# ziniuwan/maed

Measured on AMD Instinct MI355X. Metric: video-clips/sec (BxT frames) train step, higher is better.
Workload: dtype bf16

## Files before the change

include/maed_hip.h:

```cpp
#ifndef MAED_HIP_H
#define MAED_HIP_H

#include <stddef.h>
#include <stdint.h>

#ifdef __cplusplus
extern "C" {
#endif

typedef enum { MAED_F32 = 0, MAED_BF16 = 1,
               MAED_F32X3 = 2, MAED_F32X6 = 3,
               MAED_F32X1 = 4 } maed_dtype;

typedef enum {
    MAED_OK = 0,
    MAED_ERR_ARG = -1,
    MAED_ERR_SHAPE = -2,
    MAED_ERR_ALIGN = -3,
    MAED_ERR_LAUNCH = -4,
    MAED_ERR_UNSUPPORTED = -5
} maed_status;

typedef enum {
    MAED_EPI_STORE = 0,
    MAED_EPI_GELU = 1,
    MAED_EPI_RESID_F32 = 2,
    MAED_EPI_MUL_DGELU = 3,
    MAED_EPI_ATOMIC_F32 = 4,
    MAED_EPI_STORE_F32 = 5,
    MAED_EPI_TANH = 6,
    MAED_EPI_ADD = 7
} maed_epilogue;

typedef enum { MAED_IMPL_AUTO = 0, MAED_IMPL_VALU = 1, MAED_IMPL_MFMA = 2,
               MAED_IMPL_MFMA_GLDS1 = 3, MAED_IMPL_MFMA_GLDS2 = 4,
               MAED_IMPL_MFMA_LONG = 5,
               MAED_IMPL_MFMA_256 = 6,
               MAED_IMPL_X1 = 9,
               MAED_IMPL_MFMA_SK = 10,
               MAED_IMPL_X3 = 7, MAED_IMPL_X6 = 8
} maed_impl;

const char* maed_last_error(void);
int maed_version(void);

typedef enum {
    MAED_OPT_F32_MATMUL = 0,
    MAED_OPT_SIDE_STREAM = 1,
    MAED_OPT_TN_TARGET_WGS = 2,
    MAED_OPT_ABLATE = 3,
    MAED_OPT_GN_BWD_ONEPASS = 4,
    MAED_OPT_F32_BWD_X1 = 5,
    MAED_OPT_ST_FUSED = 6,
    MAED_OPT_CONV3X3_ROWS_WGS = 7,
    MAED_OPT_STEM_WGRAD_WGS = 8,
    MAED_OPT_LBS_FRAMES = 9,
    MAED_OPT_TN_DMA = 10,
    MAED_OPT_X3_PLANES = 11,
    MAED_OPT_X3_PLANES_LN = 12,
    MAED_OPT_SK = 13,
    MAED_OPT_SK_GRID = 14,
    MAED_OPT_TN_SK = 15,
    MAED_OPT_CONV3X3_NARROW_WGS = 16,
    MAED_OPT_CONV3X3_FRAME = 17,
    MAED_OPT_COUNT
} maed_option;
int maed_init(int device);
int maed_device_faults(void);
int maed_device_faults_clear(void);
int maed_set_option(int key, int value);
int maed_get_option(int key);

int maed_layernorm_fwd(const float* x, int64_t x_row_stride, const float* gamma, const float* beta,
                       void* y, int dtype, float* mean, float* rstd,
                       int64_t rows, int C, float eps, void* stream);
int maed_layernorm_bwd(const void* dy, int dtype, const float* x, int64_t x_row_stride,
                       const float* gamma, const float* mean, const float* rstd,
                       const float* dres_in, float* dx_out, void* dx_twin, float* dgamma, float* dbeta,
                       int64_t rows, int C, void* stream);

int maed_gemm_nt(const void* A, int64_t lda, const void* B, int64_t ldb,
                 int64_t M, int64_t N, int64_t K, int dtype, int epilogue,
                 const float* bias, void* out, int64_t ldo, void* out2,
                 const void* aux, int64_t ldaux, int splitk, int impl, void* stream);

int maed_gemm_nt_planes(const void* a_hi, const void* a_lo, int64_t lda, const void* b_hi, const void* b_lo, int64_t ldb, int64_t M, int64_t N, int64_t K,
                        int epilogue, const float* bias, void* out, int64_t ldo, void* out2_bf16, const void* aux, int64_t ldaux, void* out_hi, void* out_lo,
                        int variant, void* stream);
int maed_split_planes(const float* x, void* hi, void* lo, int64_t n, void* stream);

int maed_gemm_tn_wgrad(const void* Y, int64_t ldy, const void* X, int64_t ldx, int64_t M, int N, int K,
                       float* dW, int64_t ldw, float* dbias, int dtype, void* stream);

int maed_transpose_cast(const void* in, int in_dtype, int64_t ldi, int64_t M, int64_t N,
                        void* out_t, int64_t ldt, void* out_c, int64_t ldc, float* colsum,
                        int dtype, void* stream);

int maed_attn_spatial_fwd(const void* qkv, void* o, float* lse, int F, int P, int H, float scale,
                          int dtype, int impl, void* stream);
int maed_attn_spatial_bwd(const void* qkv, const void* o, const void* d_o, const float* lse,
                          void* dqkv, int accumulate, int F, int P, int H, float scale,
                          int dtype, int impl, void* stream);

int maed_attn_temporal_fwd(const void* qkv, void* o, float* lse, int F, int P, int H, int T,
                           float scale, int dtype, void* stream);
int maed_attn_temporal_bwd(const void* qkv, const void* o, const void* d_o, const float* lse,
                           void* dqkv, int accumulate, int F, int P, int H, int T, float scale,
                           int dtype, void* stream);

int maed_st_colmean(const void* x_s, const void* x_t, void* means, float* ws, int F, int P, int C, int dtype, void* stream);
int maed_st_mix_fwd(const void* x_s, const void* x_t, const float* logits, void* mix,
                    int F, int P, int C, int dtype, void* stream);
int maed_st_mix_bwd_reduce(const void* dmix, const void* x_s, const void* x_t, const float* logits,
                           void* dlogits, float* ws, int F, int P, int C, int dtype, void* stream);
int maed_st_mix_bwd_apply(const void* dmix, const float* logits, const void* dmeans, void* dx_s, void* dx_t,
                          int F, int P, int C, int dtype, void* stream);
int maed_st_fused_supported(int P, int C, int dtype);
int maed_st_fused_fwd(const void* x_s, const void* x_t, const void* w_ts, const float* b_ts, void* means, float* logits, void* mix,
                      uint32_t* sync, float* ex, int F, int P, int C, int dtype, void* stream);
int maed_st_fused_bwd(const void* dmix, const void* x_s, const void* x_t, const float* logits, const void* wt_ts, void* dlogits, void* dx_s,
                      void* dx_t, uint32_t* sync, float* ex, int F, int P, int C, int dtype, void* stream);


int maed_embed_add_fwd(const void* patch, int dtype, const float* cls, const float* pos, const float* temp,
                       float* tokens, int F, int P, int C, int T, void* stream);
int maed_embed_add_bwd(const float* dtokens, void* dpatch, int dtype, float* dpos, float* dtemp, int F, int P, int C, int T, void* stream);

int maed_dropout(const float* x, float* y, int64_t n, float p, uint64_t seed, void* stream);
typedef struct { float lr, bias_corr1, bias_corr2, reserved0; uint64_t seed; uint64_t reserved1; } maed_train_state;
int maed_dropout_dev(const float* x, float* y, int64_t n, float p, const maed_train_state* state, uint64_t call_id, void* stream);
int maed_tanh_bwd(const float* dy, const void* y, void* dx, int64_t n, int dtype, void* stream);

typedef struct {
    int F, P, C, H, T, hidden;
    int dtype;
    int impl;
    float eps;
} maed_block_dims;

typedef struct {
    const float *ln1_g, *ln1_b, *ln2_g, *ln2_b;
    const void *w_qkv, *w_ts, *w_proj, *w_fc1, *w_fc2;
    const float *b_qkv, *b_ts, *b_proj, *b_fc1, *b_fc2;
    const void *wt_qkv, *wt_ts, *wt_proj, *wt_fc1, *wt_fc2;
} maed_block_params;

typedef struct {
// ... 163 lines not shown
```

maed_amd/_lib.py:

```python
import ctypes as C
import os

HERE = os.path.dirname(os.path.abspath(__file__))
LIB_PATH = os.environ.get("MAED_HIP_LIB") or os.path.join(HERE, "libmaed_hip.so")

F32, BF16 = 0, 1
F32X3, F32X6, F32X1 = 2, 3, 4
EPI_STORE, EPI_GELU, EPI_RESID_F32, EPI_MUL_DGELU, EPI_ATOMIC_F32, EPI_STORE_F32, EPI_TANH, EPI_ADD = range(8)
IMPL_AUTO, IMPL_VALU, IMPL_MFMA = 0, 1, 2
IMPL_MFMA_256 = 6
IMPL_MFMA_LONG = 5
IMPL_MFMA_SK = 10
IMPL_X3, IMPL_X6, IMPL_X1 = 7, 8, 9
(OPT_F32_MATMUL, OPT_SIDE_STREAM, OPT_TN_TARGET_WGS, OPT_ABLATE, OPT_GN_BWD_ONEPASS, OPT_F32_BWD_X1, OPT_ST_FUSED, OPT_CONV3X3_ROWS_WGS, OPT_STEM_WGRAD_WGS,
 OPT_LBS_FRAMES, OPT_TN_DMA, OPT_X3_PLANES, OPT_X3_PLANES_LN, OPT_SK, OPT_SK_GRID, OPT_TN_SK, OPT_CONV3X3_NARROW_WGS, OPT_CONV3X3_FRAME) = range(18)

vp, i64, i32, f32 = C.c_void_p, C.c_int64, C.c_int, C.c_float


class GnAffineItem(C.Structure):
    _fields_ = [("ab", C.c_void_p), ("dgamma", C.c_void_p), ("dbeta", C.c_void_p), ("N", C.c_int), ("C", C.c_int)]


class BlockDims(C.Structure):
    _fields_ = [("F", i32), ("P", i32), ("C", i32), ("H", i32), ("T", i32), ("hidden", i32),
                ("dtype", i32), ("impl", i32), ("eps", f32)]


_PARAM_FIELDS = ["ln1_g", "ln1_b", "ln2_g", "ln2_b", "w_qkv", "w_ts", "w_proj", "w_fc1", "w_fc2",
                 "b_qkv", "b_ts", "b_proj", "b_fc1", "b_fc2", "wt_qkv", "wt_ts", "wt_proj", "wt_fc1", "wt_fc2"]
_GRAD_FIELDS = _PARAM_FIELDS[:14]


class BlockParams(C.Structure):
    _fields_ = [(n, vp) for n in _PARAM_FIELDS]


class BlockGrads(C.Structure):
    _fields_ = [(n, vp) for n in _GRAD_FIELDS]


class SmplParams(C.Structure):
    _fields_ = [(n, vp) for n in ["v_template", "shapedirs", "posedirs", "J_template", "J_shapedirs", "lbs_weights", "parents"]]


class KtdPtrs(C.Structure):
    _fields_ = [("w", vp * 26), ("b", vp * 26), ("gw", vp * 26), ("gb", vp * 26)]


class LossWeights(C.Structure):
    _fields_ = [(n, f32) for n in ["w_kp2d", "w_kp3d", "w_pose", "w_shape", "w_norm"]]


KTD_W_ANC = 3420

SIGNATURES = {
    "maed_last_error": (C.c_char_p, []),
    "maed_version": (i32, []),
    "maed_init": (i32, [i32]),
    "maed_device_faults": (i32, []),
    "maed_device_faults_clear": (i32, []),
    "maed_set_option": (i32, [i32, i32]),
    "maed_get_option": (i32, [i32]),
    "maed_layernorm_fwd": (i32, [vp, i64, vp, vp, vp, i32, vp, vp, i64, i32, f32, vp]),
    "maed_layernorm_bwd": (i32, [vp, i32, vp, i64, vp, vp, vp, vp, vp, vp, vp, vp, i64, i32, vp]),
    "maed_gemm_tn_wgrad": (i32, [vp, i64, vp, i64, i64, i32, i32, vp, i64, vp, i32, vp]),
    "maed_gemm_nt": (i32, [vp, i64, vp, i64, i64, i64, i64, i32, i32, vp, vp, i64, vp, vp, i64, i32, i32, vp]),
    "maed_transpose_cast": (i32, [vp, i32, i64, i64, i64, vp, i64, vp, i64, vp, i32, vp]),
    "maed_attn_spatial_fwd": (i32, [vp, vp, vp, i32, i32, i32, f32, i32, i32, vp]),
    "maed_attn_spatial_bwd": (i32, [vp, vp, vp, vp, vp, i32, i32, i32, i32, f32, i32, i32, vp]),
    "maed_attn_temporal_fwd": (i32, [vp, vp, vp, i32, i32, i32, i32, f32, i32, vp]),
    "maed_attn_temporal_bwd": (i32, [vp, vp, vp, vp, vp, i32, i32, i32, i32, i32, f32, i32, vp]),
    "maed_st_colmean": (i32, [vp, vp, vp, vp, i32, i32, i32, i32, vp]),
    "maed_st_mix_fwd": (i32, [vp, vp, vp, vp, i32, i32, i32, i32, vp]),
    "maed_st_mix_bwd_reduce": (i32, [vp, vp, vp, vp, vp, vp, i32, i32, i32, i32, vp]),
    "maed_st_mix_bwd_apply": (i32, [vp, vp, vp, vp, vp, i32, i32, i32, i32, vp]),
    "maed_st_fused_supported": (i32, [i32, i32, i32]),
    "maed_st_fused_fwd": (i32, [vp, vp, vp, vp, vp, vp, vp, vp, vp, i32, i32, i32, i32, vp]),
    "maed_st_fused_bwd": (i32, [vp, vp, vp, vp, vp, vp, vp, vp, vp, vp, i32, i32, i32, i32, vp]),
    "maed_embed_add_fwd": (i32, [vp, i32, vp, vp, vp, vp, i32, i32, i32, i32, vp]),
    "maed_embed_add_bwd": (i32, [vp, vp, i32, vp, vp, i32, i32, i32, i32, vp]),
    "maed_ste_block_saved_bytes": (C.c_size_t, [C.POINTER(BlockDims)]),
    "maed_ste_block_scratch_bytes": (C.c_size_t, [C.POINTER(BlockDims)]),
    "maed_gemm_nt_planes": (i32, [vp, vp, i64, vp, vp, i64, i64, i64, i64, i32, vp, vp, i64, vp, vp, i64, vp, vp, i32, vp]),
    "maed_split_planes": (i32, [vp, vp, vp, i64, vp]),
    "maed_ste_block_twin_work_bytes": (C.c_size_t, [C.POINTER(BlockDims)]),
    "maed_ste_block_fwd_twin": (i32, [C.POINTER(BlockDims), C.POINTER(BlockParams), vp, vp, vp, vp, i32, vp]),
    "maed_ste_block_twin_join": (i32, [vp]),
    "maed_ste_block_fwd": (i32, [C.POINTER(BlockDims), C.POINTER(BlockParams), vp, vp, vp, vp]),
    "maed_ste_block_infer": (i32, [C.POINTER(BlockDims), C.POINTER(BlockParams), vp, vp, vp, vp]),
    "maed_ste_block_bwd": (i32, [C.POINTER(BlockDims), C.POINTER(BlockParams), C.POINTER(BlockGrads), vp, vp, vp, vp, vp, vp, vp, vp]),
    "maed_loss_accl_fwd_bwd": (i32, [vp, vp, i32, i32, f32, vp, vp, vp]),
    "maed_dropout": (i32, [vp, vp, i64, f32, C.c_uint64, vp]),
    "maed_dropout_dev": (i32, [vp, vp, i64, f32, vp, C.c_uint64, vp]),
    "maed_tanh_bwd": (i32, [vp, vp, vp, i64, i32, vp]),
    "maed_stream_fence": (i32, [vp, vp]),
    "maed_prof_enable": (i32, [i32]),
    "maed_prof_ntags": (i32, []),
# ... 23 lines not shown
    "maed_gn_affine_grad_batch": (i32, [vp, i32, vp]),
    "maed_comm_load": (i32, [C.c_char_p]),
    "maed_comm_unique_id": (i32, [vp]),
    "maed_comm_init": (i32, [i32, i32, vp]),
    "maed_comm_allreduce_async": (i32, [vp, C.c_size_t, i32, vp]),
    "maed_comm_wait": (i32, [vp]),
    "maed_comm_world": (i32, []),
    "maed_comm_destroy": (i32, []),
    "maed_conv3x3_fwd": (i32, [vp, vp, vp, vp, i32, i32, i32, i32, i32, i32, i32, i32, i32, i32, vp, i32, i32, vp, vp]),
    "maed_conv1x1_fwd": (i32, [vp, i64, vp, i64, i64, i32, i32, vp, i64, i32, vp, i32, vp]),
    "maed_conv3x3_tapmask": (i32, [vp, i32, i32, i32, vp]),
    "maed_conv3x3_s2_dgrad": (i32, [vp, vp, vp, vp, i32, i32, i32, i32, i32, i32, i32, i32, i32, i32, vp]),
    "maed_conv3x3_s2_tables": (i32, [vp, vp, i32, i32, i32, i32, i32, i32, i32, vp]),
    "maed_conv3x3_s2_wgrad": (i32, [vp, vp, vp, vp, vp, vp, i32, i32, i32, i32, i32, i32, i32, i32, vp]),
    "maed_conv3x3_wgrad": (i32, [vp, vp, vp, vp, vp, i32, i32, i32, i32, i32, i32, vp]),
    "maed_eval_pose_errors": (i32, [vp, vp, i32, i32, vp, vp, vp, vp, vp]),
    "maed_similarity_transform": (i32, [vp, vp, i32, i32, vp, vp]),
    "maed_eval_accel": (i32, [vp, vp, i32, i32, vp, vp]),
    "maed_eval_vertex_error": (i32, [vp, vp, i32, i32, vp, vp]),
    "maed_maxpool3s2_same_fwd": (i32, [vp, vp, vp, i32, i32, i32, i32, i32, vp]),
    "maed_maxpool3s2_same_bwd": (i32, [vp, vp, vp, i32, i32, i32, i32, i32, vp]),
    "maed_stem_input": (i32, [vp, vp, i32, i32, i32, i32, i32, i32, i32, i32, i32, i32, vp]),
    "maed_conv3x3_wgrad_rows64_scratch_floats": (i32, [i32, i32, i32, i32, i32]),
    "maed_conv3x3_wgrad_rows64": (i32, [vp, vp, vp, vp, i32, i32, i32, i32, vp]),
    "maed_stem7x7s2_supported": (i32, [i32, i32]),
    "maed_stem7x7s2_fwd": (i32, [vp, vp, vp, vp, vp, i32, i32, i32, i32, vp]),
    "maed_stem7x7s2_wgrad_scratch_floats": (i32, [i32, i32, i32]),
    "maed_stem7x7s2_wgrad": (i32, [vp, vp, vp, vp, i32, i32, i32, i32, vp]),
    "maed_subsample2_fwd": (i32, [vp, vp, i32, i32, i32, i32, i32, vp]),
    "maed_subsample2_bwd": (i32, [vp, vp, i32, i32, i32, i32, i32, vp]),
    "maed_weight_refresh": (i32, [vp, i32, i32, i32, vp]),
    "maed_adam_step": (i32, [vp, vp, vp, vp, vp, i64, f32, f32, f32, f32, f32, f32, f32, f32, vp]),
    "maed_adam_step_dev": (i32, [vp, vp, vp, vp, vp, i64, vp, f32, f32, f32, f32, f32, vp]),
}

_lib = None
_init_pending = False


class MaedHipError(RuntimeError):
    pass


def lib():
    global _lib, _init_pending
    if _lib is None:
        if not os.path.exists(LIB_PATH):
            raise MaedHipError(f"{LIB_PATH} is missing: build it with `python -m maed_amd.build` "
                               "(hipcc --offload-arch=gfx950).  maed_amd has no non-HIP fallback.")
        handle = C.CDLL(LIB_PATH)
        for name, (res, args) in SIGNATURES.items():
            fn = getattr(handle, name)
            fn.restype, fn.argtypes = res, args
        _lib = handle
        apply_options(handle)
        _init_pending = True
    if _init_pending:
        import torch
        if torch.cuda.is_available() and torch.cuda.is_initialized():
            _init_pending = False
            check(_lib.maed_init(torch.cuda.current_device()), "maed_init")
    return _lib


_OPTIONS = {
    OPT_F32_MATMUL: {"exact": 0, "0": 0, "bf16x3": 1, "1": 1, "bf16x6": 2, "2": 2}[os.environ.get("MAED_F32_MATMUL", "exact")],
    OPT_SIDE_STREAM: int(os.environ.get("MAED_WGRAD_SIDE_STREAM", "1") == "1"),
    OPT_TN_TARGET_WGS: int(os.environ.get("MAED_TN_TARGET_WGS", "0")),
    OPT_ABLATE: int(os.environ.get("MAED_GEMM_ABLATE", "0")),
    OPT_F32_BWD_X1: int(os.environ.get("MAED_F32_BWD", "") == "bf16x1"),
    OPT_ST_FUSED: int(os.environ.get("MAED_ST_FUSED", "1")),
    OPT_GN_BWD_ONEPASS: int(os.environ.get("MAED_GN_BWD_ONEPASS", "1")),
    OPT_CONV3X3_ROWS_WGS: 0 if os.environ.get("MAED_CONV3X3_WGRAD_ROWS", "1") == "0" else int(os.environ.get("MAED_CONV3X3_ROWS_WGS", "256")),
    OPT_STEM_WGRAD_WGS: int(os.environ.get("MAED_STEM_WGS", "512")),
    OPT_LBS_FRAMES: int(os.environ.get("MAED_LBS_FB", "0")),
    OPT_TN_DMA: int(os.environ.get("MAED_TN_DMA", "1")),
    OPT_X3_PLANES: int(os.environ.get("MAED_X3_PLANES", "6")),
    OPT_SK: int(os.environ.get("MAED_SK", "1")),
    OPT_SK_GRID: int(os.environ.get("MAED_SK_GRID", "0")),
    OPT_CONV3X3_FRAME: int(os.environ.get("MAED_CONV3X3_FRAME", "1")),
    OPT_CONV3X3_NARROW_WGS: int(os.environ.get("MAED_CONV3X3_NARROW_WGS", "0")),
    OPT_TN_SK: int(os.environ.get("MAED_TN_SK", "1")),
    OPT_X3_PLANES_LN: int(os.environ.get("MAED_X3_PLANES_LN", "0")),
}


def apply_options(handle):
    for k, v in _OPTIONS.items():
        if handle.maed_set_option(k, v) != 0:
            raise MaedHipError(f"maed_set_option({k}, {v}) failed")


def set_option(key, value):
    _OPTIONS[key] = int(value)
    if _lib is not None:
        check(_lib.maed_set_option(key, int(value)), "set_option")


def get_option(key):
    return _OPTIONS[key]


def check(rc, what=""):
    if rc != 0:
        msg = lib().maed_last_error().decode("utf-8", "replace")
        raise MaedHipError(f"{what or 'libmaed_hip'} failed with status {rc}: {msg}")


def device_faults():
    return 0 if _lib is None else int(_lib.maed_device_faults())


def loaded_path():
    return LIB_PATH if _lib is not None else None
```

maed_amd/csrc/gemm.hip:

```cpp
#include "common.cuh"
#include "gemm_epilogue.cuh"
#include "gemm_x3.h"

template <int EPI, typename T>
__global__ __launch_bounds__(256) void gemm_nt_valu_kernel(const T* __restrict__ A, int64_t lda, const T* __restrict__ B,
                                                           int64_t ldb, int64_t M, int64_t N, int64_t K, int64_t k_per_split,
                                                           EpiArgs e) {
    __shared__ float As[16][64 + 1];
    __shared__ float Bs[16][64 + 1];
    const int tid = threadIdx.x;
    const int64_t m0 = (int64_t)blockIdx.y * 64, n0 = (int64_t)blockIdx.x * 64;
    const int64_t kbeg = (int64_t)blockIdx.z * k_per_split;
    const int64_t kend = (kbeg + k_per_split < K) ? kbeg + k_per_split : K;
    const int ty = tid >> 4, tx = tid & 15;
    const int lr = tid >> 2, lk = (tid & 3) * 4;
    float acc[4][4];
#pragma unroll
    for (int i = 0; i < 4; ++i)
#pragma unroll
        for (int j = 0; j < 4; ++j) acc[i][j] = 0.f;
    const int64_t ar = (m0 + lr < M) ? m0 + lr : M - 1;
    const int64_t br = (n0 + lr < N) ? n0 + lr : N - 1;
    const bool vec = sizeof(T) == 4 && (lda % 4 == 0) && (ldb % 4 == 0) && (((uintptr_t)A | (uintptr_t)B) & 15) == 0 && (kbeg % 4 == 0);
    float va[4], vb[4];
// ... 595 lines not shown
    MAED_CHECK_ARG(is_aligned(dy, 16) && is_aligned(wt_image, 16) && is_aligned(zero_page, 16) && is_aligned(dx, 16), MAED_ERR_ALIGN, "conv3x3_s2_dgrad: 16-B alignment");
    MAED_CHECK_ARG((uint64_t)F * H * W * Cin * 2 < (1ull << 32) && (uint64_t)F * Ho * Wo * Cout * 2 < (1ull << 32), MAED_ERR_SHAPE, "conv3x3_s2_dgrad: tensor larger than 4 GB");
    if (F == 0) return MAED_OK;
    const int64_t N = Cin;
    const bool narrow = N <= 64;
    const int tn = narrow ? 1 : (int)((N + GM_BN - 1) / GM_BN);
    EpiArgs e{nullptr, dx, (int64_t)Cin, nullptr, nullptr, (int64_t)Cin};
    for (int py = 0; py < 2; ++py)
        for (int px = 0; px < 2; ++px) {
            const int Ha = (H - py + 1) / 2, Wb = (W - px + 1) / 2;
            if (Ha <= 0 || Wb <= 0) continue;
            const int ey = (py + pad_top) & 1, ex = (px + pad_left) & 1;
            const int nty = ey ? 1 : 2, ntx = ex ? 1 : 2;
            const int base_y = (py + pad_top - ey) / 2 - (nty - 1), base_x = (px + pad_left - ex) / 2 - (ntx - 1);
            Conv3x3Dims d{F, Ho, Wo, Cout, Ha, Wb, 1, -base_y, -base_x, (int64_t)Cout, (int64_t)Cin * Cout, 0};
            d.nty = nty; d.ntx = ntx; d.ky0 = ey + 2 * (nty - 1); d.kx0 = ex + 2 * (ntx - 1); d.o_h = H; d.o_w = W; d.o_py = py; d.o_px = px;
            const int64_t M = (int64_t)F * Ha * Wb;
            const dim3 grid((unsigned)(((M + GM_BM - 1) / GM_BM) * tn));
            if (narrow) hipLaunchKernelGGL((conv3x3_glds_bf16_kernel<MAED_EPI_STORE, true, false, true>), grid, dim3(256), 0, (hipStream_t)stream, (const bf16*)dy,
                                           (const bf16*)wt_image, (const bf16*)zero_page, d, M, N, tn, e);
            else hipLaunchKernelGGL((conv3x3_glds_bf16_kernel<MAED_EPI_STORE, false, false, true>), grid, dim3(256), 0, (hipStream_t)stream, (const bf16*)dy,
                                    (const bf16*)wt_image, (const bf16*)zero_page, d, M, N, tn, e);
        }
    MAED_CHECK_LAUNCH("conv3x3_s2_dgrad");
    return MAED_OK;
}

__global__ __launch_bounds__(256) void bias_fill_kernel(float* __restrict__ out, int64_t ldo, const float* __restrict__ bias, int64_t M, int64_t N) {
    const int64_t i = (int64_t)blockIdx.x * 256 + threadIdx.x;
    if (i < M * N) { const int64_t r = i / N, c = i % N; out[r * ldo + c] = bias ? bias[c] : 0.f; }
}

template <int EPI, typename T>
static int launch_valu(const void* A, int64_t lda, const void* B, int64_t ldb, int64_t M, int64_t N, int64_t K,
                       const EpiArgs& e, int splitk, hipStream_t s) {
    int64_t kps = (K + splitk - 1) / splitk;
    kps = (kps + 15) / 16 * 16;
    const int z = (int)((K + kps - 1) / kps);
    dim3 grid((unsigned)((N + 63) / 64), (unsigned)((M + 63) / 64), (unsigned)z);
    hipLaunchKernelGGL((gemm_nt_valu_kernel<EPI, T>), grid, dim3(256), 0, s, (const T*)A, lda, (const T*)B, ldb, M, N, K, kps, e);
    return MAED_OK;
}

template <int EPI>
static int launch_mfma(const void* A, int64_t lda, const void* B, int64_t ldb, int64_t M, int64_t N, int64_t K,
                       const EpiArgs& e, int splitk, hipStream_t s) {
    const int tm = (int)((M + GM_BM - 1) / GM_BM), tn = (int)((N + GM_BN - 1) / GM_BN);
    const int nkt = (int)(K / GM_BK);
    int kps = (nkt + splitk - 1) / splitk;
    if (kps < 1) kps = 1;
    const int z = (nkt + kps - 1) / kps;
    dim3 grid((unsigned)(tm * tn), 1, (unsigned)z);
    hipLaunchKernelGGL((gemm_nt_mfma_bf16_kernel<EPI>), grid, dim3(256), 0, s, (const bf16*)A, lda, (const bf16*)B, ldb,
                       M, N, K, tn, kps, e);
    return MAED_OK;
}

template <int EPI, int NBUF, bool GN = false>
static int launch_glds(const void* A, int64_t lda, const void* B, int64_t ldb, int64_t M, int64_t N, int64_t K,
                       const EpiArgs& e, int splitk, hipStream_t s) {
    const int tm = (int)((M + GM_BM - 1) / GM_BM), tn = (int)((N + GM_BN - 1) / GM_BN);
    const int nkt = (int)(K / GM_BK);
    int kps = (nkt + splitk - 1) / splitk;
    if (kps < 1) kps = 1;
    const int z = (nkt + kps - 1) / kps;
#ifdef MAED_GEMM_ABLATE
    hipLaunchKernelGGL((gemm_nt_glds_bf16_kernel<EPI, NBUF, GN>), dim3((unsigned)(tm * tn), 1, (unsigned)z), dim3(256), 0, s, (const bf16*)A, lda,
                       (const bf16*)B, ldb, M, N, K, tn, kps, e, maed_opt(MAED_OPT_ABLATE));
#else
    hipLaunchKernelGGL((gemm_nt_glds_bf16_kernel<EPI, NBUF, GN>), dim3((unsigned)(tm * tn), 1, (unsigned)z), dim3(256), 0, s, (const bf16*)A, lda,
                       (const bf16*)B, ldb, M, N, K, tn, kps, e);
#endif
    return MAED_OK;
}

bool maed_gemm_nt_256_launch(int epilogue, const void* A, int64_t lda, const void* B, int64_t ldb, int64_t M, int64_t N, int64_t K, const EpiArgs& e,
                             hipStream_t s);

bool maed_gemm_nt_sk_shape_ok(int64_t M, int64_t N, int64_t K);
bool maed_gemm_nt_sk_launch(int epilogue, const void* A, int64_t lda, const void* B, int64_t ldb, int64_t M, int64_t N, int64_t K, const EpiArgs& e,
                            int mode, int grid_opt, hipStream_t s);
int maed_sk_cus(void);

template <int EPI>
static int dispatch(const void* A, int64_t lda, const void* B, int64_t ldb, int64_t M, int64_t N, int64_t K, int dtype,
                    const EpiArgs& e, int splitk, int impl, hipStream_t s) {
    if (dtype == MAED_F32) {
        MAED_CHECK_ARG(impl == MAED_IMPL_AUTO || impl == MAED_IMPL_VALU || impl == MAED_IMPL_X3 || impl == MAED_IMPL_X6 || impl == MAED_IMPL_X1, MAED_ERR_UNSUPPORTED,
                       "gemm_nt: f32 runs on the exact-f32 VALU kernel (MAED_IMPL_VALU) or the split-bf16 MFMA kernel (MAED_IMPL_X3 / _X6); impl=%d", impl);
        const int np = impl == MAED_IMPL_X3 ? 2 : impl == MAED_IMPL_X6 ? 3 : impl == MAED_IMPL_X1 ? 1 : impl == MAED_IMPL_AUTO ? maed_x3_planes() : 0;
        if (np) {
            const bool ok = maed_x3_nt_shape_ok(A, lda, B, ldb, K);
            const int64_t tiles128 = ((M + 127) / 128) * ((N + 127) / 128);
            if constexpr (EPI == MAED_EPI_STORE || EPI == MAED_EPI_STORE_F32) {
                if (ok && impl != MAED_IMPL_AUTO && splitk == 1 && tiles128 < 48 && K >= 256 && e.ldo >= N && !e.twin && !e.lo && !e.out2_bf16) {
                    int sk = (int)(256 / tiles128);
                    if (sk > K / 32) sk = (int)(K / 32);
                    if (sk > 1) {
                        hipLaunchKernelGGL(bias_fill_kernel, dim3((unsigned)((M * N + 255) / 256)), dim3(256), 0, s, (float*)e.out, e.ldo, e.bias, M, N);
                        EpiArgs ea = e;
                        ea.bias = nullptr;
                        return maed_gemm_nt_x3_launch(MAED_EPI_ATOMIC_F32, np, A, lda, B, ldb, M, N, K, ea, sk, s);
                    }
                }
            }
            if (ok && (impl != MAED_IMPL_AUTO || tiles128 >= 48 || EPI == MAED_EPI_ATOMIC_F32))
                return maed_gemm_nt_x3_launch(EPI, np, A, lda, B, ldb, M, N, K, e, splitk, s);
        }
        if constexpr (EPI == MAED_EPI_STORE || EPI == MAED_EPI_STORE_F32) {
            const int64_t tiles = ((M + 63) / 64) * ((N + 63) / 64);
            if (splitk == 1 && tiles < 96 && K >= 256 && !e.twin && !e.lo && !e.out2_bf16) {
                constexpr int target = 256;
                int sk = (int)(target / tiles);
                if (sk > K / 64) sk = (int)(K / 64);
                if (sk > 1) {
                    hipLaunchKernelGGL(bias_fill_kernel, dim3((unsigned)((M * N + 255) / 256)), dim3(256), 0, s, (float*)e.out, e.ldo, e.bias, M, N);
                    EpiArgs ea{nullptr, e.out, e.ldo, nullptr, nullptr, 0};
                    if (np && maed_x3_nt_shape_ok(A, lda, B, ldb, K)) {
                        const int64_t t128 = ((M + 127) / 128) * ((N + 127) / 128);
                        int sk3 = (int)(256 / t128);
                        if (sk3 > K / 64) sk3 = (int)(K / 64);
                        if (sk3 >= 1) return maed_gemm_nt_x3_launch(MAED_EPI_ATOMIC_F32, np, A, lda, B, ldb, M, N, K, ea, sk3, s);
                    }
                    return launch_valu<MAED_EPI_ATOMIC_F32, float>(A, lda, B, ldb, M, N, K, ea, sk, s);
                }
            }
        }
        return launch_valu<EPI, float>(A, lda, B, ldb, M, N, K, e, splitk, s);
    }
    const bool fits32 = (uint64_t)M * (uint64_t)lda * 2 < (1ull << 32) && (uint64_t)N * (uint64_t)ldb * 2 < (1ull << 32);
    const bool mfma_ok = (K % GM_BK == 0) && (lda % 8 == 0) && (ldb % 8 == 0) && is_aligned(A, 16) && is_aligned(B, 16);
    if (impl == MAED_IMPL_VALU) return launch_valu<EPI, bf16>(A, lda, B, ldb, M, N, K, e, splitk, s);
    if (impl == MAED_IMPL_MFMA_GLDS1 || impl == MAED_IMPL_MFMA_GLDS2) {
        MAED_CHECK_ARG(mfma_ok && fits32, MAED_ERR_ALIGN, "gemm_nt(glds): need K%%64==0 (K=%lld), lda/ldb%%8==0, 16-B aligned A/B", (long long)K);
        return impl == MAED_IMPL_MFMA_GLDS1 ? launch_glds<EPI, 1>(A, lda, B, ldb, M, N, K, e, splitk, s)
                                            : launch_glds<EPI, 2>(A, lda, B, ldb, M, N, K, e, splitk, s);
    }
    const bool ok256 = mfma_ok && fits32 && K >= 128 && splitk == 1 && EPI != MAED_EPI_ATOMIC_F32;
    if (impl == MAED_IMPL_MFMA_256) {
        MAED_CHECK_ARG(ok256, MAED_ERR_ALIGN, "gemm_nt(256): need K%%64==0, K>=128 (K=%lld), lda/ldb%%8==0, 16-B aligned A/B, no split-K", (long long)K);
        maed_gemm_nt_256_launch(EPI, A, lda, B, ldb, M, N, K, e, s);
        return MAED_OK;
    }
    const bool oksk = ok256 && maed_gemm_nt_sk_shape_ok(M, N, K) && !e.gn_sums;
    if (impl == MAED_IMPL_MFMA_SK) {
        const int mode = maed_opt(MAED_OPT_SK);
        MAED_CHECK_ARG(oksk && maed_gemm_nt_sk_launch(EPI, A, lda, B, ldb, M, N, K, e, mode == 0 ? 1 : mode, maed_opt(MAED_OPT_SK_GRID), s), MAED_ERR_ALIGN,
                       "gemm_nt(sk): need K%%128==0 (K=%lld), M, N >= 256, lda/ldb%%8==0, 16-B aligned A/B, no split-K, the library's slab allocation", (long long)K);
        return MAED_OK;
    }
    if (impl == MAED_IMPL_MFMA) {
        MAED_CHECK_ARG(mfma_ok, MAED_ERR_ALIGN, "gemm_nt(mfma): need K%%64==0 (K=%lld), lda/ldb%%8==0, 16-B aligned A/B", (long long)K);
        return launch_mfma<EPI>(A, lda, B, ldb, M, N, K, e, splitk, s);
    }
    if (!mfma_ok) return launch_valu<EPI, bf16>(A, lda, B, ldb, M, N, K, e, splitk, s);
    if constexpr (EPI != MAED_EPI_ATOMIC_F32) {
        const int64_t tiles256 = ((M + 255) / 256) * ((N + 255) / 256);
        const int skmode = maed_opt(MAED_OPT_SK);
        if (oksk && skmode != 0 && tiles256 * 10 >= (int64_t)maed_sk_cus() * 7 &&
            maed_gemm_nt_sk_launch(EPI, A, lda, B, ldb, M, N, K, e, skmode, maed_opt(MAED_OPT_SK_GRID), s))
            return MAED_OK;
        if (ok256 && N >= 256 && tiles256 >= 180 && (K >= 1024 || tiles256 <= 256)) {
            maed_gemm_nt_256_launch(EPI, A, lda, B, ldb, M, N, K, e, s);
            return MAED_OK;
        }
    }
    if constexpr (EPI == MAED_EPI_ATOMIC_F32) return launch_mfma<EPI>(A, lda, B, ldb, M, N, K, e, splitk, s);
    else return fits32 ? launch_glds<EPI, 1>(A, lda, B, ldb, M, N, K, e, splitk, s) : launch_mfma<EPI>(A, lda, B, ldb, M, N, K, e, splitk, s);
}

extern "C" int maed_conv1x1_fwd(const void* x, int64_t ldx, const void* w, int64_t ldw, int64_t M, int Cout, int Cin, void* y, int64_t ldy, int hw,
                                double* gn_sums, int dtype, void* stream) {
    MAED_CHECK_ARG(x && w && y, MAED_ERR_ARG, "conv1x1_fwd: null pointer");
    const int np_call = maed_x3_take_dtype(dtype);
    MAED_CHECK_ARG(dtype == MAED_BF16 || dtype == MAED_F32, MAED_ERR_ARG, "conv1x1_fwd: bad dtype %d", dtype);
    MAED_CHECK_ARG(is_aligned(x, 16) && is_aligned(w, 16) && is_aligned(y, 16), MAED_ERR_ALIGN, "conv1x1_fwd: 16-B alignment");
    MAED_CHECK_ARG(!gn_sums || gn_stats_shape_ok(Cout, hw), MAED_ERR_SHAPE, "conv1x1_fwd: GroupNorm statistics need Cout = 32 * 2^k >= 64 and hw >= 128 (Cout=%d hw=%d)", Cout, hw);
    EpiArgs e{nullptr, y, ldy, nullptr, nullptr, 0, gn_sums, hw};
    if (dtype == MAED_F32) {
        const int x3np = np_call ? np_call : maed_x3_planes();
        MAED_CHECK_ARG(x3np, MAED_ERR_UNSUPPORTED, "conv1x1_fwd: f32 needs the split-bf16 matmul mode (maed_set_option(MAED_OPT_F32_MATMUL, 1 or 2))");
        MAED_CHECK_ARG(M >= 0 && Cout > 0 && Cin > 0 && ldx >= Cin && ldw >= Cin && ldy >= Cout && ldy % 4 == 0 && maed_x3_nt_shape_ok(x, ldx, w, ldw, Cin), MAED_ERR_SHAPE,
                       "conv1x1_fwd(f32): need Cin %% 32 == 0 and 4-element aligned strides (Cin=%d Cout=%d)", Cin, Cout);
        if (M == 0) return MAED_OK;
        MAED_PROPAGATE(maed_conv1x1_x3_launch(x3np, x, ldx, w, ldw, M, Cout, Cin, e, gn_sums != nullptr, (hipStream_t)stream));
        MAED_CHECK_LAUNCH("conv1x1_fwd(x3)");
        return MAED_OK;
    }
    MAED_CHECK_ARG(M >= 0 && Cout > 0 && Cin > 0 && Cin % GM_BK == 0 && ldx >= Cin && ldw >= Cin && ldy >= Cout && ldx % 8 == 0 && ldw % 8 == 0, MAED_ERR_SHAPE,
                   "conv1x1_fwd: need Cin %% 64 == 0 and 8-element aligned strides (Cin=%d Cout=%d)", Cin, Cout);
    MAED_CHECK_ARG((uint64_t)M * (uint64_t)ldx * 2 < (1ull << 32), MAED_ERR_SHAPE, "conv1x1_fwd: activation larger than 4 GB");
    if (M == 0) return MAED_OK;
    if (gn_sums) launch_glds<MAED_EPI_STORE, 1, true>(x, ldx, w, ldw, M, Cout, Cin, e, 1, (hipStream_t)stream);
    else launch_glds<MAED_EPI_STORE, 1>(x, ldx, w, ldw, M, Cout, Cin, e, 1, (hipStream_t)stream);
    MAED_CHECK_LAUNCH("conv1x1_fwd");
    return MAED_OK;
}

int maed_gemm_nt_twin(const void* A, int64_t lda, const void* B, int64_t ldb, int64_t M, int64_t N, int64_t K,
                      int dtype, int epilogue, const float* bias, void* out, int64_t ldo, void* out2,
                      const void* aux, int64_t ldaux, int splitk, int impl, void* stream, void* twin, bool out2_bf16, void* lo);
extern "C" int maed_gemm_nt(const void* A, int64_t lda, const void* B, int64_t ldb, int64_t M, int64_t N, int64_t K,
                            int dtype, int epilogue, const float* bias, void* out, int64_t ldo, void* out2,
                            const void* aux, int64_t ldaux, int splitk, int impl, void* stream) {
    return maed_gemm_nt_twin(A, lda, B, ldb, M, N, K, dtype, epilogue, bias, out, ldo, out2, aux, ldaux, splitk, impl, stream, nullptr, false, nullptr);
}
int maed_gemm_nt_twin(const void* A, int64_t lda, const void* B, int64_t ldb, int64_t M, int64_t N, int64_t K,
                      int dtype, int epilogue, const float* bias, void* out, int64_t ldo, void* out2,
                      const void* aux, int64_t ldaux, int splitk, int impl, void* stream, void* twin, bool out2_bf16, void* lo) {
    MAED_CHECK_ARG(A && B && (out || (twin && lo)), MAED_ERR_ARG, "gemm_nt: null pointer");
    MAED_CHECK_ARG(!lo || (twin && is_aligned(lo, 16)), MAED_ERR_ARG, "gemm_nt: a lo plane goes with the twin (hi) plane, 16-byte aligned");
    {
        const int np_call = maed_x3_take_dtype(dtype);
        if (np_call && impl == MAED_IMPL_AUTO) impl = np_call == 2 ? MAED_IMPL_X3 : np_call == 1 ? MAED_IMPL_X1 : MAED_IMPL_X6;
    }
    MAED_CHECK_ARG(dtype == MAED_F32 || dtype == MAED_BF16, MAED_ERR_ARG, "gemm_nt: bad dtype %d", dtype);
    MAED_CHECK_ARG(M >= 0 && N > 0 && K > 0 && lda >= K && ldb >= K && ldo >= N, MAED_ERR_SHAPE, "gemm_nt: bad extents M=%lld N=%lld K=%lld", (long long)M, (long long)N, (long long)K);
    if (splitk < 1) splitk = 1;
    MAED_CHECK_ARG(splitk == 1 || epilogue == MAED_EPI_ATOMIC_F32, MAED_ERR_ARG, "gemm_nt: split-K needs the atomic epilogue");
    if (M == 0) return MAED_OK;
    MAED_CHECK_ARG(!(twin || out2_bf16) || (dtype == MAED_F32 && (epilogue == MAED_EPI_STORE || epilogue == MAED_EPI_GELU) && N % 8 == 0 && ldo % 8 == 0
                                           && is_aligned(twin, 16) && (!out2_bf16 || is_aligned(out2, 16))),
                   MAED_ERR_ARG, "gemm_nt: twin outputs go with fp32 operands, the STORE / GELU epilogues, N and ldo multiples of 8 and 16-byte aligned buffers");
    EpiArgs e{bias, out, ldo, out2, aux, ldaux};
    e.twin = twin; e.out2_bf16 = out2_bf16; e.lo = lo;
    hipStream_t s = (hipStream_t)stream;
    int rc;
    switch (epilogue) {
        case MAED_EPI_STORE: rc = dispatch<MAED_EPI_STORE>(A, lda, B, ldb, M, N, K, dtype, e, splitk, impl, s); break;
        case MAED_EPI_GELU:
            rc = dispatch<MAED_EPI_GELU>(A, lda, B, ldb, M, N, K, dtype, e, splitk, impl, s); break;
        case MAED_EPI_RESID_F32:
            MAED_CHECK_ARG(aux, MAED_ERR_ARG, "gemm_nt: RESID epilogue needs aux");
            rc = dispatch<MAED_EPI_RESID_F32>(A, lda, B, ldb, M, N, K, dtype, e, splitk, impl, s); break;
        case MAED_EPI_MUL_DGELU:
            MAED_CHECK_ARG(aux, MAED_ERR_ARG, "gemm_nt: MUL_DGELU epilogue needs aux");
            rc = dispatch<MAED_EPI_MUL_DGELU>(A, lda, B, ldb, M, N, K, dtype, e, splitk, impl, s); break;
        case MAED_EPI_ATOMIC_F32: rc = dispatch<MAED_EPI_ATOMIC_F32>(A, lda, B, ldb, M, N, K, dtype, e, splitk, impl, s); break;
// ... 12 lines not shown
```

maed_amd/csrc/options.hip:

```cpp
#include "common.cuh"
#include "gemm_x3.h"
#include <atomic>
#include <string.h>

static std::atomic<int> g_opt[MAED_OPT_COUNT] = {
    {0},
    {1},
    {0},
    {0},
    {1},
    {0},
    {1},
    {256},
    {512},
    {0},
    {1},
    {6},
    {0},
    {1},
    {0},
    {1},
    {0},
    {1},
};

extern "C" int maed_init(int device) {
#ifndef MAED_HOSTSIM
    hipDeviceProp_t prop;
    if (hipGetDeviceProperties(&prop, device) != hipSuccess) { (void)hipGetLastError(); maed_set_error("init: no HIP device %d", device); return MAED_ERR_ARG; }
    if (!strstr(prop.gcnArchName, "gfx950")) {
        maed_set_error("init: device %d is %s; libmaed_hip is built for gfx950 (MI355X) only", device, prop.gcnArchName);
        return MAED_ERR_UNSUPPORTED;
    }
#else
    (void)device;
#endif
    (void)maed_fault_word();
#ifndef MAED_HOSTSIM
    if (maed_init_runtime() != MAED_OK) { maed_set_error("init: could not create the library's side streams / event rings"); return MAED_ERR_LAUNCH; }
#endif
    return MAED_OK;
}

static std::atomic<uint32_t*> g_fault{nullptr};
static std::atomic<int> g_fault_told{0};
uint32_t* maed_fault_word(void) {
    uint32_t* w = g_fault.load(std::memory_order_acquire);
    if (w) return w;
#ifdef MAED_HOSTSIM
    uint32_t* n = (uint32_t*)calloc(16, sizeof(uint32_t));
#else
    uint32_t* n = nullptr;
    if (hipHostMalloc((void**)&n, 64, hipHostMallocMapped | hipHostMallocCoherent) != hipSuccess || !n) { (void)hipGetLastError(); return nullptr; }
    memset(n, 0, 64);
#endif
    uint32_t* expected = nullptr;
    if (!g_fault.compare_exchange_strong(expected, n, std::memory_order_acq_rel)) {
#ifdef MAED_HOSTSIM
        free(n);
#else
        (void)hipHostFree(n);
#endif
        return expected;
    }
    return n;
}
bool maed_fault_seen(const char* who) {
    uint32_t* w = g_fault.load(std::memory_order_acquire);
    if (!w || *(volatile uint32_t*)w == 0) return false;
    if (!g_fault_told.exchange(1))
        maed_set_error("%s: %u frame-barrier timeout(s) on this device (workgroups of a frame were not co-resident: shared GPU / preemption); the affected results were "
                       "NaN-poisoned, the one-pass GroupNorm backward and the fused attentive addition now run as their multi-launch forms", who, *(volatile uint32_t*)w);
    return true;
}
extern "C" int maed_device_faults(void) {
    uint32_t* w = g_fault.load(std::memory_order_acquire);
    const int n = w ? (int)*(volatile uint32_t*)w : 0;
    if (n > 0)
        maed_set_error("%d frame-barrier timeout(s) on this device (workgroups of a frame were not co-resident: shared GPU / preemption); the affected results were "
                       "NaN-poisoned, the one-pass GroupNorm backward and the fused attentive addition run as their multi-launch forms from the next call on", n);
    return n;
}
extern "C" int maed_device_faults_clear(void) { uint32_t* w = g_fault.load(std::memory_order_acquire); if (w) *(volatile uint32_t*)w = 0; g_fault_told.store(0); return MAED_OK; }

extern "C" int maed_set_option(int key, int value) {
    MAED_CHECK_ARG(key >= 0 && key < MAED_OPT_COUNT, MAED_ERR_ARG, "set_option: unknown option %d", key);
    if (key == MAED_OPT_F32_MATMUL) MAED_CHECK_ARG(value >= 0 && value <= 2, MAED_ERR_ARG, "set_option: MAED_OPT_F32_MATMUL takes 0 (exact), 1 (bf16x3) or 2 (bf16x6)");
    if (key == MAED_OPT_TN_TARGET_WGS) MAED_CHECK_ARG(value == 0 || value >= 64, MAED_ERR_ARG, "set_option: MAED_OPT_TN_TARGET_WGS must be 0 (heuristic) or >= 64");
    if (key == MAED_OPT_CONV3X3_ROWS_WGS || key == MAED_OPT_STEM_WGRAD_WGS) MAED_CHECK_ARG(value >= 0 && value <= 65535, MAED_ERR_ARG, "set_option: workgroup count out of range");
    if (key == MAED_OPT_LBS_FRAMES) MAED_CHECK_ARG(value == 0 || value == 4 || value == 8 || value == 16, MAED_ERR_ARG, "set_option: MAED_OPT_LBS_FRAMES takes 0 (auto), 4, 8 or 16");
    if (key == MAED_OPT_X3_PLANES) MAED_CHECK_ARG(value == 0 || (value >= 2 && value <= 7 && value != 3), MAED_ERR_ARG, "set_option: MAED_OPT_X3_PLANES takes 0 (fp32 operands) or a kernel variant 2, 4, 5, 6, 7");
    if (key == MAED_OPT_SK) MAED_CHECK_ARG(value >= 0 && value <= 3, MAED_ERR_ARG, "set_option: MAED_OPT_SK takes 0 (off), 1 (heuristic), 2 (no K cuts) or 3 (always)");
    if (key == MAED_OPT_TN_SK) MAED_CHECK_ARG(value == 0 || value == 1, MAED_ERR_ARG, "set_option: MAED_OPT_TN_SK takes 0 or 1");
    if (key == MAED_OPT_SK_GRID) MAED_CHECK_ARG(value >= 0 && value <= 512, MAED_ERR_ARG, "set_option: MAED_OPT_SK_GRID takes 0 (one workgroup per CU) or a workgroup count <= 512");
    g_opt[key].store(value, std::memory_order_relaxed);
    return MAED_OK;
}

extern "C" int maed_get_option(int key) {
    if (key < 0 || key >= MAED_OPT_COUNT) { maed_set_error("get_option: unknown option %d", key); return MAED_ERR_ARG; }
    return g_opt[key].load(std::memory_order_relaxed);
}

int maed_opt(int key) { return g_opt[key].load(std::memory_order_relaxed); }

int maed_x3_planes(void) {
    const int v = maed_opt(MAED_OPT_F32_MATMUL);
    return v == 1 ? 2 : v == 2 ? 3 : 0;
}
```

Measured before the change: 409.7.

## Add persistent panel GEMM kernel keeping A K-panel resident in LDS

Adds a persistent MFMA bf16 NT GEMM. Each workgroup owns a contiguous run of 128x128 output tiles and keeps the full A row-panel (K up to 512) in LDS, so A is loaded once per tile row while B slices stream through a 4-deep DMA ring. It is selected automatically for short-K GEMMs with simple epilogues when there are at least as many tiles as CUs. The aim is to cut redundant A global loads and launch/tail overhead for the transformer's small-K matmuls, at the cost of large LDS use (one workgroup per CU) and possible load imbalance.

```diff
diff --git a/include/maed_hip.h b/include/maed_hip.h
--- a/include/maed_hip.h
+++ b/include/maed_hip.h
@@ -38,6 +38,7 @@
                MAED_IMPL_MFMA_256 = 6,
                MAED_IMPL_X1 = 9,
                MAED_IMPL_MFMA_SK = 10,
+               MAED_IMPL_MFMA_PANEL = 11,
                MAED_IMPL_X3 = 7, MAED_IMPL_X6 = 8
 } maed_impl;
 
@@ -63,6 +64,7 @@
     MAED_OPT_TN_SK = 15,
     MAED_OPT_CONV3X3_NARROW_WGS = 16,
     MAED_OPT_CONV3X3_FRAME = 17,
+    MAED_OPT_GEMM_PANEL = 18,
     MAED_OPT_COUNT
 } maed_option;
 int maed_init(int device);
diff --git a/maed_amd/_lib.py b/maed_amd/_lib.py
--- a/maed_amd/_lib.py
+++ b/maed_amd/_lib.py
@@ -11,9 +11,11 @@
 IMPL_MFMA_256 = 6
 IMPL_MFMA_LONG = 5
 IMPL_MFMA_SK = 10
+IMPL_MFMA_PANEL = 11
 IMPL_X3, IMPL_X6, IMPL_X1 = 7, 8, 9
 (OPT_F32_MATMUL, OPT_SIDE_STREAM, OPT_TN_TARGET_WGS, OPT_ABLATE, OPT_GN_BWD_ONEPASS, OPT_F32_BWD_X1, OPT_ST_FUSED, OPT_CONV3X3_ROWS_WGS, OPT_STEM_WGRAD_WGS,
- OPT_LBS_FRAMES, OPT_TN_DMA, OPT_X3_PLANES, OPT_X3_PLANES_LN, OPT_SK, OPT_SK_GRID, OPT_TN_SK, OPT_CONV3X3_NARROW_WGS, OPT_CONV3X3_FRAME) = range(18)
+ OPT_LBS_FRAMES, OPT_TN_DMA, OPT_X3_PLANES, OPT_X3_PLANES_LN, OPT_SK, OPT_SK_GRID, OPT_TN_SK, OPT_CONV3X3_NARROW_WGS, OPT_CONV3X3_FRAME,
+ OPT_GEMM_PANEL) = range(19)
 
 vp, i64, i32, f32 = C.c_void_p, C.c_int64, C.c_int, C.c_float
 
@@ -203,6 +205,7 @@
     OPT_CONV3X3_NARROW_WGS: int(os.environ.get("MAED_CONV3X3_NARROW_WGS", "0")),
     OPT_TN_SK: int(os.environ.get("MAED_TN_SK", "1")),
     OPT_X3_PLANES_LN: int(os.environ.get("MAED_X3_PLANES_LN", "0")),
+    OPT_GEMM_PANEL: int(os.environ.get("MAED_GEMM_PANEL", "1")),
 }
 
 
diff --git a/maed_amd/csrc/gemm.hip b/maed_amd/csrc/gemm.hip
--- a/maed_amd/csrc/gemm.hip
+++ b/maed_amd/csrc/gemm.hip
@@ -701,6 +701,8 @@
                             int mode, int grid_opt, hipStream_t s);
 int maed_sk_cus(void);
 
+#include "gemm_panel.cuh"
+
 template <int EPI>
 static int dispatch(const void* A, int64_t lda, const void* B, int64_t ldb, int64_t M, int64_t N, int64_t K, int dtype,
                     const EpiArgs& e, int splitk, int impl, hipStream_t s) {
@@ -768,11 +770,18 @@
                        "gemm_nt(sk): need K%%128==0 (K=%lld), M, N >= 256, lda/ldb%%8==0, 16-B aligned A/B, no split-K, the library's slab allocation", (long long)K);
         return MAED_OK;
     }
+    if (impl == MAED_IMPL_MFMA_PANEL) {
+        MAED_CHECK_ARG(launch_panel<EPI>(A, lda, B, ldb, M, N, K, e, splitk, 2, s), MAED_ERR_ALIGN,
+                       "gemm_nt(panel): need the STORE / GELU / RESID_F32 / MUL_DGELU epilogue without twins or statistics, K%%64==0 and 128 <= K <= 512 (K=%lld), "
+                       "lda/ldb%%8==0, 16-B aligned A/B, no split-K", (long long)K);
+        return MAED_OK;
+    }
     if (impl == MAED_IMPL_MFMA) {
         MAED_CHECK_ARG(mfma_ok, MAED_ERR_ALIGN, "gemm_nt(mfma): need K%%64==0 (K=%lld), lda/ldb%%8==0, 16-B aligned A/B", (long long)K);
         return launch_mfma<EPI>(A, lda, B, ldb, M, N, K, e, splitk, s);
     }
     if (!mfma_ok) return launch_valu<EPI, bf16>(A, lda, B, ldb, M, N, K, e, splitk, s);
+    if (impl == MAED_IMPL_AUTO && launch_panel<EPI>(A, lda, B, ldb, M, N, K, e, splitk, maed_opt(MAED_OPT_GEMM_PANEL), s)) return MAED_OK;
     if constexpr (EPI != MAED_EPI_ATOMIC_F32) {
         const int64_t tiles256 = ((M + 255) / 256) * ((N + 255) / 256);
         const int skmode = maed_opt(MAED_OPT_SK);
diff --git a/maed_amd/csrc/gemm_panel.cuh b/maed_amd/csrc/gemm_panel.cuh
--- /dev/null
+++ b/maed_amd/csrc/gemm_panel.cuh
@@ -0,0 +1,172 @@
+#pragma once
+
+#define GP_BM 128
+#define GP_BN 128
+#define GP_BK 32
+#define GP_SLICE (GP_BM * GP_BK)
+#define GP_KMAX 512
+#define GP_NS 4
+#define GP_B_OFF ((GP_KMAX / GP_BK) * GP_SLICE)
+
+template <int EPI>
+__global__ __launch_bounds__(256, 1) void gemm_nt_panel_bf16_kernel(const bf16* __restrict__ A, int64_t lda, const bf16* __restrict__ B, int64_t ldb,
+                                                                    int64_t M, int64_t N, int64_t K, int tiles_n, int ntiles, EpiArgs e
+#ifdef MAED_GEMM_ABLATE
+                                                                    , int ablate
+#endif
+                                                                    ) {
+#ifndef MAED_GEMM_ABLATE
+    constexpr int ablate = 0;
+#endif
+    __shared__ __attribute__((aligned(1024))) unsigned short lds[GP_B_OFF + GP_NS * GP_SLICE];
+    const int tid = threadIdx.x, lane = tid & 63;
+    const int wave = __builtin_amdgcn_readfirstlane(tid >> 6);
+    const int wr = wave >> 1, wc = wave & 1;
+    const int l31 = lane & 31, hi = lane >> 5;
+    const int nwg = gridDim.x, id = xcd_remap(blockIdx.x, nwg);
+    const int per = ntiles / nwg, rem = ntiles % nwg;
+    const int t_beg = id * per + (id < rem ? id : rem);
+    const int cnt = per + (id < rem ? 1 : 0);
+    if (cnt == 0) return;
+    const int S = (int)(K / GP_BK);
+    const int nsl = cnt * S;
+
+    const int drow = lane >> 2;
+    const int dchunk = ((lane & 3) ^ ((lane >> 4) & 3)) * 8;
+    const char* const Ab = reinterpret_cast<const char*>(A);
+    const char* const Bb = reinterpret_cast<const char*>(B);
+    int itm = t_beg / tiles_n, itn = t_beg % tiles_n, is = 0, ig = 0;
+    auto issue_next = [&]() -> int {
+        const int64_t m0 = (int64_t)itm * GP_BM, n0 = (int64_t)itn * GP_BN;
+        const char* const bk = Bb + (int64_t)is * (GP_BK * 2);
+        unsigned short* const bslot = &lds[GP_B_OFF + (ig & (GP_NS - 1)) * GP_SLICE];
+#pragma unroll
+        for (int i = 0; i < 2 && !(ablate & 2); ++i) {
+            const int row = (4 * i + wave) * 16 + drow;
+            const int64_t br = (n0 + row < N) ? n0 + row : N - 1;
+            MAED_LDS_DMA16(bk, (uint32_t)((br * ldb + dchunk) * 2), bslot + (4 * i + wave) * 16 * GP_BK);
+        }
+        const bool with_a = ig < S || itn == 0;
+        if (with_a && !(ablate & 2)) {
+            const char* const ak = Ab + (int64_t)is * (GP_BK * 2);
+            unsigned short* const aimg = &lds[is * GP_SLICE];
+#pragma unroll
+            for (int i = 0; i < 2; ++i) {
+                const int row = (4 * i + wave) * 16 + drow;
+                const int64_t ar = (m0 + row < M) ? m0 + row : M - 1;
+                MAED_LDS_DMA16(ak, (uint32_t)((ar * lda + dchunk) * 2), aimg + (4 * i + wave) * 16 * GP_BK);
+            }
+        }
+        ++ig;
+        if (++is == S) { is = 0; if (++itn == tiles_n) { itn = 0; ++itm; } }
+        return with_a ? 4 : 2;
+    };
+
+    const int fsw = (l31 >> 2) & 3;
+    const bool vec_ok = (e.ldo % 4 == 0) && (e.ldaux % 4 == 0);
+    issue_next();
+    int o1 = 1 < nsl ? issue_next() : 0;
+    int o2 = 2 < nsl ? issue_next() : 0;
+    int g = 0;
+    int ctm = t_beg / tiles_n, ctn = t_beg % tiles_n;
+    for (int t = 0; t < cnt; ++t) {
+        f32x16_t acc00, acc01, acc10, acc11;
+#pragma unroll
+        for (int r = 0; r < 16; ++r) { acc00[r] = 0.f; acc01[r] = 0.f; acc10[r] = 0.f; acc11[r] = 0.f; }
+        for (int s = 0; s < S; ++s, ++g) {
+            switch (o1 + o2) {
+                case 8: MAED_WAIT_VMCNT(8); break;
+                case 6: MAED_WAIT_VMCNT(6); break;
+                case 4: MAED_WAIT_VMCNT(4); break;
+                case 2: MAED_WAIT_VMCNT(2); break;
+                default: MAED_WAIT_VMCNT0(); break;
+            }
+            MAED_WAIT_LGKMCNT0();
+            __builtin_amdgcn_sched_barrier(0);
+            __builtin_amdgcn_s_barrier();
+            __builtin_amdgcn_sched_barrier(0);
+            const unsigned short* As = &lds[s * GP_SLICE + (wr * 64 + l31) * GP_BK];
+            const unsigned short* Bs = &lds[GP_B_OFF + (g & (GP_NS - 1)) * GP_SLICE + (wc * 64 + l31) * GP_BK];
+            bf16x8_t a0[2], a1[2], b0[2], b1[2];
+#pragma unroll
+            for (int kk = 0; kk < 2; ++kk) {
+                const int co = ((kk * 2 + hi) ^ fsw) * 8;
+                a0[kk] = *reinterpret_cast<const bf16x8_t*>(As + co);
+                a1[kk] = *reinterpret_cast<const bf16x8_t*>(As + 32 * GP_BK + co);
+                b0[kk] = *reinterpret_cast<const bf16x8_t*>(Bs + co);
+                b1[kk] = *reinterpret_cast<const bf16x8_t*>(Bs + 32 * GP_BK + co);
+            }
+            __builtin_amdgcn_sched_barrier(0);
+            const int o3 = g + 3 < nsl ? issue_next() : 0;
+            __builtin_amdgcn_sched_barrier(0);
+#pragma unroll
+            for (int kk = 0; kk < 2 && !(ablate & 4); ++kk) {
+                acc00 = __builtin_amdgcn_mfma_f32_32x32x16_bf16(b0[kk], a0[kk], acc00, 0, 0, 0);
+                acc01 = __builtin_amdgcn_mfma_f32_32x32x16_bf16(b1[kk], a0[kk], acc01, 0, 0, 0);
+                acc10 = __builtin_amdgcn_mfma_f32_32x32x16_bf16(b0[kk], a1[kk], acc10, 0, 0, 0);
+                acc11 = __builtin_amdgcn_mfma_f32_32x32x16_bf16(b1[kk], a1[kk], acc11, 0, 0, 0);
+            }
+            o1 = o2; o2 = o3;
+        }
+        const int64_t m0 = (int64_t)ctm * GP_BM, n0 = (int64_t)ctn * GP_BN;
+        if (++ctn == tiles_n) { ctn = 0; ++ctm; }
+#define GP_EPILOGUE(acc_, i_, j_)                                                                         \
+        {                                                                                                 \
+            const int64_t row = m0 + wr * 64 + (i_) * 32 + l31;                                           \
+            if (row < M) {                                                                                \
+                _Pragma("unroll") for (int q = 0; q < 4; ++q) {                                           \
+                    const int64_t c0 = n0 + wc * 64 + (j_) * 32 + 8 * q + 4 * hi;                         \
+                    const float v4[4] = {acc_[4 * q], acc_[4 * q + 1], acc_[4 * q + 2], acc_[4 * q + 3]}; \
+                    if (c0 < N) epilogue_store4<EPI, bf16>(e, row, c0, N, v4, vec_ok);                    \
+                }                                                                                         \
+            }                                                                                             \
+        }
+        if (!(ablate & 1)) {
+            GP_EPILOGUE(acc00, 0, 0)
+            GP_EPILOGUE(acc01, 0, 1)
+            GP_EPILOGUE(acc10, 1, 0)
+            GP_EPILOGUE(acc11, 1, 1)
+        }
+#undef GP_EPILOGUE
+    }
+}
+
+template <int EPI>
+static bool gemm_panel_epilogue_ok(const EpiArgs& e) {
+    return (EPI == MAED_EPI_STORE || EPI == MAED_EPI_GELU || EPI == MAED_EPI_RESID_F32 || EPI == MAED_EPI_MUL_DGELU) && !e.gn_sums && !e.twin && !e.lo && !e.out2_bf16;
+}
+
+static int gemm_panel_cus() {
+#ifdef MAED_HOSTSIM
+    return 8;
+#else
+    static const int n = [] {
+        int dev = 0, cus = 0;
+        if (hipGetDevice(&dev) != hipSuccess || hipDeviceGetAttribute(&cus, hipDeviceAttributeMultiprocessorCount, dev) != hipSuccess) { (void)hipGetLastError(); return 0; }
+        return cus;
+    }();
+    return n;
+#endif
+}
+
+template <int EPI>
+static bool launch_panel(const void* A, int64_t lda, const void* B, int64_t ldb, int64_t M, int64_t N, int64_t K, const EpiArgs& e, int splitk, int mode,
+                         hipStream_t s) {
+    if constexpr (!(EPI == MAED_EPI_STORE || EPI == MAED_EPI_GELU || EPI == MAED_EPI_RESID_F32 || EPI == MAED_EPI_MUL_DGELU)) return false;
+    else {
+    const int cus = gemm_panel_cus();
+    if (mode == 0 || cus <= 0 || splitk != 1 || !gemm_panel_epilogue_ok<EPI>(e)) return false;
+    if (K % 64 != 0 || K < 4 * GP_BK || K > GP_KMAX || lda % 8 != 0 || ldb % 8 != 0 || !is_aligned(A, 16) || !is_aligned(B, 16)) return false;
+    if (!((uint64_t)M * (uint64_t)lda * 2 < (1ull << 32) && (uint64_t)N * (uint64_t)ldb * 2 < (1ull << 32))) return false;
+    const int64_t tiles = ((M + GP_BM - 1) / GP_BM) * ((N + GP_BN - 1) / GP_BN);
+    if (tiles >= (1ll << 30) || (mode == 1 && tiles < cus)) return false;
+    const int grid = tiles < cus ? (int)tiles : cus;
+    hipLaunchKernelGGL((gemm_nt_panel_bf16_kernel<EPI>), dim3((unsigned)grid), dim3(256), 0, s, (const bf16*)A, lda, (const bf16*)B, ldb, M, N, K,
+                       (int)((N + GP_BN - 1) / GP_BN), (int)tiles, e
+#ifdef MAED_GEMM_ABLATE
+                       , maed_opt(MAED_OPT_ABLATE)
+#endif
+                       );
+    return true;
+    }
+}
diff --git a/maed_amd/csrc/options.hip b/maed_amd/csrc/options.hip
--- a/maed_amd/csrc/options.hip
+++ b/maed_amd/csrc/options.hip
@@ -21,6 +21,7 @@
     {0},
     {1},
     {0},
+    {1},
     {1},
 };
 
@@ -91,6 +92,7 @@
     if (key == MAED_OPT_LBS_FRAMES) MAED_CHECK_ARG(value == 0 || value == 4 || value == 8 || value == 16, MAED_ERR_ARG, "set_option: MAED_OPT_LBS_FRAMES takes 0 (auto), 4, 8 or 16");
     if (key == MAED_OPT_X3_PLANES) MAED_CHECK_ARG(value == 0 || (value >= 2 && value <= 7 && value != 3), MAED_ERR_ARG, "set_option: MAED_OPT_X3_PLANES takes 0 (fp32 operands) or a kernel variant 2, 4, 5, 6, 7");
     if (key == MAED_OPT_SK) MAED_CHECK_ARG(value >= 0 && value <= 3, MAED_ERR_ARG, "set_option: MAED_OPT_SK takes 0 (off), 1 (heuristic), 2 (no K cuts) or 3 (always)");
+    if (key == MAED_OPT_GEMM_PANEL) MAED_CHECK_ARG(value >= 0 && value <= 2, MAED_ERR_ARG, "set_option: MAED_OPT_GEMM_PANEL takes 0 (never), 1 (auto) or 2 (whenever the shape allows)");
     if (key == MAED_OPT_TN_SK) MAED_CHECK_ARG(value == 0 || value == 1, MAED_ERR_ARG, "set_option: MAED_OPT_TN_SK takes 0 or 1");
     if (key == MAED_OPT_SK_GRID) MAED_CHECK_ARG(value >= 0 && value <= 512, MAED_ERR_ARG, "set_option: MAED_OPT_SK_GRID takes 0 (one workgroup per CU) or a workgroup count <= 512");
     g_opt[key].store(value, std::memory_order_relaxed);
```

New measurement: 373.1 (median of 2 runs). -8.9%, worse.
